# huttered40/capital

Hardware: AMD Instinct MI355X
Metric: TFLOP/s (whole node) Cholesky n=65536, algorithmic n^3/3, recursive cholinv factor(), inputs resident in HBM (higher is better)
Workload: dtype f64

## Files before the change

capital_amd/csrc/equil_f64.hip:

```cpp
#include <float.h>
#include <limits.h>

#include "capi_internal.h"
#include "thin_tile.h"

namespace {

namespace tt = thin_tile;
using tt::d2_t;

__device__ __forceinline__ int scale_exponent(double s) { return (int)((__double_as_longlong(s) >> 52) & 0x7ff) - 1023; }

constexpr int PQ_THREADS = 1024;

__device__ __forceinline__ int frexp_exponent(double a) {
  const unsigned long long b = (unsigned long long)__double_as_longlong(a);
  const int E = (int)((b >> 52) & 0x7ff);
  if (E != 0) return E - 1022;
  return (63 - __clzll((long long)(b & 0xfffffffffffffULL))) - 1073;
}

__global__ __launch_bounds__(PQ_THREADS) void poequ2_kernel(int64_t n, const double* __restrict__ A, int64_t lda, double* __restrict__ dscale,
                                                            double* __restrict__ rec) {
  __shared__ int s_emin[16], s_emax[16];
  __shared__ double s_amin[16], s_amax[16];
  __shared__ long long s_bad[16];
  const int tid = threadIdx.x, lane = tid & 63, w = tid >> 6;
  int emin = INT_MAX, emax = INT_MIN;
  double amin = DBL_MAX, amax = 0.0;
  long long bad = LLONG_MAX;
  for (int64_t j = tid; j < n; j += PQ_THREADS) {
    const double a = A[j + j * lda];
    if (!(a > 0.0) || !(a <= DBL_MAX)) { bad = bad < j ? bad : (long long)j; continue; }
    const int e = frexp_exponent(a) >> 1;
    emin = e < emin ? e : emin; emax = e > emax ? e : emax;
    amin = a < amin ? a : amin; amax = a > amax ? a : amax;
  }
#pragma unroll
  for (int d = 1; d < 64; d <<= 1) {
    const int e0 = __shfl_xor(emin, d), e1 = __shfl_xor(emax, d);
    const double a0 = __shfl_xor(amin, d), a1 = __shfl_xor(amax, d);
    const long long b = __shfl_xor(bad, d);
    emin = e0 < emin ? e0 : emin; emax = e1 > emax ? e1 : emax;
    amin = a0 < amin ? a0 : amin; amax = a1 > amax ? a1 : amax;
    bad = b < bad ? b : bad;
  }
  if (lane == 0) { s_emin[w] = emin; s_emax[w] = emax; s_amin[w] = amin; s_amax[w] = amax; s_bad[w] = bad; }
  __syncthreads();
  for (int k = 0; k < 16; ++k) {
    emin = s_emin[k] < emin ? s_emin[k] : emin; emax = s_emax[k] > emax ? s_emax[k] : emax;
    amin = s_amin[k] < amin ? s_amin[k] : amin; amax = s_amax[k] > amax ? s_amax[k] : amax;
    bad = s_bad[k] < bad ? s_bad[k] : bad;
  }
  const bool ok = bad == LLONG_MAX;
  for (int64_t j = tid; j < n; j += PQ_THREADS) {
    double s = 1.0;
    if (ok) s = __longlong_as_double((long long)((frexp_exponent(A[j + j * lda]) >> 1) + 1023) << 52);
    dscale[j] = s;
  }
  if (tid == 0) {
    rec[0] = ok ? ldexp(1.0, emin - emax) : 1.0;
    rec[1] = ok ? amax : 0.0;
    rec[2] = ok ? amin : 0.0;
    rec[3] = ok ? 0.0 : (double)(bad + 1);
  }
}

constexpr int SC_THREADS = 256;
constexpr int SC_ROWS = 512, SC_COLS = 64, SC_PASS = 8;
constexpr int SC_K = SC_ROWS / SC_COLS;

__host__ __device__ inline int64_t tiles_before(int64_t J) {
  const int64_t q = J / SC_K, s = J % SC_K;
  return SC_K * q * (q + 1) / 2 + s * (q + 1);
}

template <bool VEC>
__global__ __launch_bounds__(SC_THREADS) void sym_scale2_kernel(int64_t n, double* __restrict__ A, int64_t lda, const double* __restrict__ dscale, int sign) {
  const int tid = threadIdx.x;
  const int64_t t = blockIdx.x;
  int64_t q = (int64_t)((sqrt(1.0 + 8.0 * (double)t / SC_K) - 1.0) * 0.5);
  while (q > 0 && SC_K * q * (q + 1) / 2 > t) --q;
  while (SC_K * (q + 1) * (q + 2) / 2 <= t) ++q;
  const int64_t rem = t - SC_K * q * (q + 1) / 2;
  const int64_t J = SC_K * q + rem / (q + 1), I = rem % (q + 1);
  const int64_t i0 = I * SC_ROWS, j0 = J * SC_COLS;
  const bool whole = i0 + SC_ROWS <= j0 + 1 && j0 + SC_COLS <= n;
  if (whole) {
    if (VEC) {
      const int64_t i = i0 + 2 * tid;
      const int ei0 = scale_exponent(dscale[i]), ei1 = scale_exponent(dscale[i + 1]);
      for (int64_t c = j0; c < j0 + SC_COLS; c += SC_PASS) {
        d2_t v[SC_PASS];
#pragma unroll
        for (int p = 0; p < SC_PASS; ++p) v[p] = *(const d2_t*)(A + i + (c + p) * lda);
#pragma unroll
        for (int p = 0; p < SC_PASS; ++p) {
          const int ej = scale_exponent(dscale[c + p]);
          v[p].x = ldexp(v[p].x, -sign * (ei0 + ej));
          v[p].y = ldexp(v[p].y, -sign * (ei1 + ej));
        }
#pragma unroll
        for (int p = 0; p < SC_PASS; ++p) *(d2_t*)(A + i + (c + p) * lda) = v[p];
      }
    } else {
      const int64_t i = i0 + tid;
      const int ei0 = scale_exponent(dscale[i]), ei1 = scale_exponent(dscale[i + SC_THREADS]);
      for (int64_t c = j0; c < j0 + SC_COLS; c += SC_PASS) {
        double x[SC_PASS], y[SC_PASS];
#pragma unroll
        for (int p = 0; p < SC_PASS; ++p) { x[p] = A[i + (c + p) * lda]; y[p] = A[i + SC_THREADS + (c + p) * lda]; }
#pragma unroll
        for (int p = 0; p < SC_PASS; ++p) {
          const int ej = scale_exponent(dscale[c + p]);
          x[p] = ldexp(x[p], -sign * (ei0 + ej));
          y[p] = ldexp(y[p], -sign * (ei1 + ej));
        }
#pragma unroll
        for (int p = 0; p < SC_PASS; ++p) { A[i + (c + p) * lda] = x[p]; A[i + SC_THREADS + (c + p) * lda] = y[p]; }
      }
    }
    return;
  }
  const int64_t ra = i0 + tid, rb = ra + SC_THREADS;
  const int ea = scale_exponent(dscale[ra < n ? ra : 0]), eb = scale_exponent(dscale[rb < n ? rb : 0]);
  for (int64_t c = j0; c < j0 + SC_COLS && c < n; c += SC_PASS) {
    if (i0 + (tid & ~63) > c + SC_PASS - 1) continue;
    double x[SC_PASS], y[SC_PASS];
    bool va[SC_PASS], vb[SC_PASS];
#pragma unroll
    for (int p = 0; p < SC_PASS; ++p) {
      const int64_t col = c + p;
      va[p] = col < n && ra <= col;
      vb[p] = col < n && rb <= col;
      x[p] = *(va[p] ? A + ra + col * lda : A);
      y[p] = *(vb[p] ? A + rb + col * lda : A);
    }
#pragma unroll
    for (int p = 0; p < SC_PASS; ++p) {
      const int ej = scale_exponent(dscale[c + p < n ? c + p : 0]);
      x[p] = ldexp(x[p], -sign * (ea + ej));
      y[p] = ldexp(y[p], -sign * (eb + ej));
    }
#pragma unroll
    for (int p = 0; p < SC_PASS; ++p) {
      if (va[p]) A[ra + (c + p) * lda] = x[p];
      if (vb[p]) A[rb + (c + p) * lda] = y[p];
    }
  }
}

constexpr int RS_THREADS = 256;

__global__ __launch_bounds__(RS_THREADS) void row_scale2_kernel(int64_t m, const double* __restrict__ dscale, int sign, const double* X, int64_t ldx, double* Y,
                                                                int64_t ldy, double* __restrict__ norm2) {
  __shared__ double red[4];
  const double* x = X + (int64_t)blockIdx.x * ldx;
  double* y = Y + (int64_t)blockIdx.x * ldy;
  double s = 0.0;
  for (int64_t i = threadIdx.x; i < m; i += RS_THREADS) {
    const double v = ldexp(x[i], sign * scale_exponent(dscale[i]));
    y[i] = v;
    s += v * v;
  }
  if (!norm2) return;
  s = tt::butterfly_sum<64>(s);
  if ((threadIdx.x & 63) == 0) red[threadIdx.x >> 6] = s;
  __syncthreads();
  if (threadIdx.x == 0) norm2[blockIdx.x] = ((red[0] + red[1]) + red[2]) + red[3];
}

}

extern "C" {

int capi_dpoequ2(capi_handle_t h, int64_t n, const double* A, int64_t lda, double* dscale, double* rec) {
  CAPI_REQUIRE(h, h, "null handle");
  CAPI_REQUIRE(h, n >= 0 && n < (1LL << 31), "n");
  if (n == 0) return CAPI_OK;
  CAPI_REQUIRE(h, A && lda >= n && dscale && rec, "A / lda >= n / dscale / rec");
  hipLaunchKernelGGL(poequ2_kernel, dim3(1), dim3(PQ_THREADS), 0, h->stream, n, A, lda, dscale, rec);
  CAPI_HIP_CHECK(h, hipGetLastError());
  return CAPI_OK;
}

int capi_dsym_scale2(capi_handle_t h, int64_t n, double* A, int64_t lda, const double* dscale, int sign) {
  CAPI_REQUIRE(h, h, "null handle");
  CAPI_REQUIRE(h, n >= 0 && n < (1LL << 31), "n");
  CAPI_REQUIRE(h, sign == 1 || sign == -1, "sign: +1 scales, -1 undoes");
  if (n == 0) return CAPI_OK;
  CAPI_REQUIRE(h, A && lda >= n && dscale, "A / lda >= n / dscale");
  const int64_t tiles = tiles_before(cdiv(n, SC_COLS));
  CAPI_REQUIRE(h, tiles < (1LL << 31), "n too large");
  const bool vec = ((uintptr_t)A & 15) == 0 && (lda & 1) == 0;
  if (vec) hipLaunchKernelGGL(sym_scale2_kernel<true>, dim3((unsigned)tiles), dim3(SC_THREADS), 0, h->stream, n, A, lda, dscale, sign);
  else hipLaunchKernelGGL(sym_scale2_kernel<false>, dim3((unsigned)tiles), dim3(SC_THREADS), 0, h->stream, n, A, lda, dscale, sign);
  CAPI_HIP_CHECK(h, hipGetLastError());
  return CAPI_OK;
}

int capi_drow_scale2(capi_handle_t h, int64_t m, int64_t r, const double* dscale, int sign, const double* X, int64_t ldx, double* Y, int64_t ldy, double* norm2) {
  CAPI_REQUIRE(h, h, "null handle");
  CAPI_REQUIRE(h, m >= 0 && r >= 0 && r < (1LL << 31), "m / r");
  CAPI_REQUIRE(h, sign == 1 || sign == -1, "sign: +1 multiplies by dscale, -1 divides");
  if (r == 0 || m == 0) return CAPI_OK;
  CAPI_REQUIRE(h, dscale && X && Y && ldx >= m && ldy >= m, "dscale / X / Y / ldx >= m / ldy >= m");
  hipLaunchKernelGGL(row_scale2_kernel, dim3((unsigned)r), dim3(RS_THREADS), 0, h->stream, m, dscale, sign, X, ldx, Y, ldy, norm2);
  CAPI_HIP_CHECK(h, hipGetLastError());
  return CAPI_OK;
}

}
```

capital_amd/csrc/movement.hip:

```cpp
#include "capi_internal.h"

namespace {

__device__ __host__ inline int64_t st_offset(int st, int64_t x, int64_t y, int64_t dimY) {
  if (st == CAPI_RECT) return x * dimY + y;
  if (st == CAPI_UPPERTRI) return ((x * (x + 1)) >> 1) + y;
  return x * dimY + y - (x * (x + 1) / 2);
}

__global__ void serialize_kernel(int shape, int ss, int ds, const double* __restrict__ src, int64_t sdimY, double* __restrict__ dst,
                                 int64_t ddimY, int64_t ssx, int64_t ssy, int64_t dsx, int64_t dsy, int64_t rangeX,
                                 int64_t rangeY) {
  const int64_t y = (int64_t)blockIdx.x * 1024 + threadIdx.x;
  const bool lower = shape == CAPI_LOWERTRI, upper = shape == CAPI_UPPERTRI;
  for (int64_t i = blockIdx.y; i < rangeX; i += gridDim.y) {
    int64_t so, d_o, cnt;
    if (lower) {
      so = st_offset(ss, ssx + i, ssy + i, sdimY);
      d_o = st_offset(ds, dsx + i, dsy + i, ddimY);
      cnt = rangeY - i;
    } else {
      so = st_offset(ss, ssx + i, ssy, sdimY);
      d_o = st_offset(ds, dsx + i, dsy, ddimY);
      cnt = upper ? i + 1 : rangeY;
    }
    if (y >= cnt) continue;
    double v[4];
#pragma unroll
    for (int q = 0; q < 4; ++q) v[q] = src[so + (y + 256 * q < cnt ? y + 256 * q : y)];
#pragma unroll
    for (int q = 0; q < 4; ++q)
      if (y + 256 * q < cnt) dst[d_o + y + 256 * q] = v[q];
  }
}

__global__ void lacpy_kernel(int part, int64_t m, int64_t n, const double* __restrict__ A, int64_t lda, double* __restrict__ B,
                             int64_t ldb) {
  const int64_t i = (int64_t)blockIdx.x * blockDim.x + threadIdx.x;
  const int64_t j0 = (int64_t)blockIdx.y * 8;
  if (i >= m) return;
#pragma unroll
  for (int q = 0; q < 8; ++q) {
    const int64_t j = j0 + q;
    if (j >= n) break;
    if (part == 1 && i > j) continue;
    if (part == 2 && i < j) continue;
    B[i + j * ldb] = A[i + j * lda];
  }
}

typedef double d2m_t __attribute__((ext_vector_type(2)));
template <bool VEC>
__global__ __launch_bounds__(256) void copy2d_kernel(int64_t m, int64_t n, const double* __restrict__ A, int64_t lda, double* __restrict__ B, int64_t ldb) {
  const int64_t i = ((int64_t)blockIdx.x * 256 + threadIdx.x) * (VEC ? 2 : 1);
  if (i >= m) return;
  for (int64_t j0 = (int64_t)blockIdx.y * 8; j0 < n; j0 += (int64_t)gridDim.y * 8) {
    if (VEC) {
      d2m_t v[8];
#pragma unroll
      for (int q = 0; q < 8; ++q) v[q] = *(const d2m_t*)(A + i + (j0 + q < n ? j0 + q : j0) * lda);
#pragma unroll
      for (int q = 0; q < 8; ++q)
        if (j0 + q < n) *(d2m_t*)(B + i + (j0 + q) * ldb) = v[q];
    } else {
      double v[8];
#pragma unroll
      for (int q = 0; q < 8; ++q) v[q] = A[i + (j0 + q < n ? j0 + q : j0) * lda];
#pragma unroll
      for (int q = 0; q < 8; ++q)
        if (j0 + q < n) B[i + (j0 + q) * ldb] = v[q];
    }
  }
}

__global__ void geadd_kernel(int part, int64_t m, int64_t n, double alpha, const double* __restrict__ X, int64_t ldx, double beta,
                             double* __restrict__ Y, int64_t ldy) {
  const int64_t i = (int64_t)blockIdx.x * blockDim.x + threadIdx.x;
  if (i >= m) return;
  for (int64_t j = blockIdx.y; j < n; j += gridDim.y) {
    if (part == 1 && i > j) continue;
    if (part == 2 && i < j) continue;
    const double x = alpha == 0.0 ? 0.0 : alpha * X[i + j * ldx];
    Y[i + j * ldy] = beta == 0.0 ? x : x + beta * Y[i + j * ldy];
  }
}

__global__ void trizero_kernel(int keep_uplo, int64_t n, double* __restrict__ A, int64_t lda) {
  const int64_t i = (int64_t)blockIdx.x * blockDim.x + threadIdx.x;
  if (i >= n) return;
  for (int64_t j = blockIdx.y; j < n; j += gridDim.y)
    if (keep_uplo == CAPI_UPPER ? (i > j) : (i < j)) A[i + j * lda] = 0.0;
}

__global__ void axpby_kernel(int64_t count, double beta, const double* __restrict__ x, double* __restrict__ y) {
  int64_t i = (int64_t)blockIdx.x * blockDim.x + threadIdx.x;
  const int64_t stride = (int64_t)gridDim.x * blockDim.x;
  for (; i < count; i += stride) y[i] = beta * y[i] + x[i];
}

__global__ void remove_triangle_kernel(int dirU, double* __restrict__ A, int64_t dimX, int64_t dimY, int64_t px, int64_t py,
                                       int64_t P) {
  const int64_t j = (int64_t)blockIdx.x * blockDim.x + threadIdx.x;
  if (j >= dimY) return;
  for (int64_t i = blockIdx.y; i < dimX; i += gridDim.y) {
    const int64_t gx = px + i * P, gy = py + j * P;
    if (dirU ? (gy > gx) : (gy < gx)) A[i * dimY + j] = 0.0;
  }
}

__global__ void block_cyclic_kernel(int to_cyclic, double* __restrict__ blocked, double* __restrict__ cyclic, int64_t rl,
                                    int64_t cl, int64_t d) {
  const int64_t grow = (int64_t)blockIdx.x * blockDim.x + threadIdx.x;
  const int64_t rg = rl * d, cg = cl * d;
  if (grow >= rg) return;
  for (int64_t gcol = blockIdx.y; gcol < cg; gcol += gridDim.y) {
    const int64_t i = gcol / d, x = gcol % d, k = grow / d, y = grow % d;
    const int64_t b = (y * d + x) * rl * cl + i * rl + k;
    if (to_cyclic == 2) cyclic[gcol * rg + grow] = blocked[b];
    else if (to_cyclic) cyclic[gcol * rg + grow] = (grow > gcol) ? 0.0 : blocked[b];
    else blocked[b] = cyclic[gcol * rg + grow];
  }
}

__global__ void block_cyclic_tri_kernel(int to_cyclic, double* __restrict__ blocked, double* __restrict__ cyclic, int64_t rl, int64_t d) {
  const int64_t grow = (int64_t)blockIdx.x * blockDim.x + threadIdx.x;
  const int64_t rg = rl * d, psz = rl * (rl + 1) / 2;
  if (grow >= rg) return;
  for (int64_t gcol = blockIdx.y; gcol < rg; gcol += gridDim.y) {
    const int64_t i = gcol / d, x = gcol % d, k = grow / d, y = grow % d;
    if (k > i) { if (to_cyclic) cyclic[gcol * rg + grow] = 0.0; continue; }
    const int64_t b = (y * d + x) * psz + i * (i + 1) / 2 + k;
    const bool below = grow > gcol;
    if (to_cyclic) cyclic[gcol * rg + grow] = below ? 0.0 : blocked[b];
    else blocked[b] = below ? 0.0 : cyclic[gcol * rg + grow];
  }
}

__global__ void cyclic_to_local_kernel(int pass, double* __restrict__ T, double* __restrict__ TI, double* __restrict__ tmp, int64_t L, int64_t bc,
                                       int64_t d, int64_t ro, int64_t co) {
  const int64_t j = (int64_t)blockIdx.x * blockDim.x + threadIdx.x;
  if (j >= L) return;
  for (int64_t i = blockIdx.y; i < L; i += gridDim.y) {
    const int64_t rc = i * d + co, rr = j * d + ro;
    if (pass == 0) {
      tmp[i * L + j] = rc >= rr ? T[rc * bc + rr] : 0.0;
      tmp[L * L + i * L + j] = rc >= rr ? TI[rc * bc + rr] : 0.0;
    } else {
      T[i * bc + j] = tmp[i * L + j];
      TI[i * bc + j] = tmp[L * L + i * L + j];
    }
  }
}

constexpr uint64_t LCG_A = 0x5DEECE66DULL, LCG_C = 0xBULL, LCG_MASK = (1ULL << 48) - 1;

__device__ __forceinline__ uint64_t seed48(int64_t seed) { return ((((uint64_t)seed) & 0xffffffffULL) << 16) | 0x330EULL; }
__device__ __forceinline__ double to_unit(uint64_t x) { return (double)x * 0x1p-48; }

__global__ void gen_symmetric_kernel(double* __restrict__ data, int64_t dimX, int64_t dimY, int64_t gdimX, int64_t gdimY,
                                     int64_t px, int64_t py, int64_t PX, int64_t PY, int64_t padX, int64_t padY, int dd) {
  const int64_t j = (int64_t)blockIdx.x * blockDim.x + threadIdx.x;
  if (j >= dimY) return;
  for (int64_t i = blockIdx.y; i < dimX; i += gridDim.y) {
    double v = 0.0;
    if (i < padX && j < padY) {
      const int64_t gx = px + i * PX, gy = py + j * PY;
      const int64_t seed = gx > gy ? gx + gdimY * gy : gy + gdimY * gx;
      const uint64_t x1 = (LCG_A * seed48(seed) + LCG_C) & LCG_MASK;
      v = to_unit(x1);
      if (dd && gx == gy && i == j) v += (double)gdimX;
    }
    data[i * dimY + j] = v;
  }
}

constexpr int GEN_CHUNK = 32;
__global__ void gen_random_kernel(double* __restrict__ data, int64_t dimX, int64_t dimY, int64_t padX, int64_t padY, int64_t key) {
  const int64_t chunk = (int64_t)blockIdx.x * blockDim.x + threadIdx.x;
  const int64_t total = padX * padY;
  int64_t t0 = chunk * GEN_CHUNK;
  if (t0 >= total) return;
  uint64_t An = 1, Cn = 0, Ab = LCG_A, Cb = LCG_C;
  for (uint64_t n = (uint64_t)t0; n; n >>= 1) {
    if (n & 1) { An = (Ab * An) & LCG_MASK; Cn = (Ab * Cn + Cb) & LCG_MASK; }
    Cb = (Ab * Cb + Cb) & LCG_MASK;
    Ab = (Ab * Ab) & LCG_MASK;
  }
  uint64_t x = (An * seed48(key) + Cn) & LCG_MASK;
  const int64_t t1 = (t0 + GEN_CHUNK < total) ? t0 + GEN_CHUNK : total;
  for (int64_t t = t0; t < t1; ++t) {
    x = (LCG_A * x + LCG_C) & LCG_MASK;
    const int64_t i = t / padY, j = t - i * padY;
    data[i * dimY + j] = to_unit(x);
  }
}

__global__ void gen_pad_zero_kernel(double* __restrict__ data, int64_t dimX, int64_t dimY, int64_t padX, int64_t padY) {
  const int64_t j = (int64_t)blockIdx.x * blockDim.x + threadIdx.x;
  if (j >= dimY) return;
  for (int64_t i = blockIdx.y; i < dimX; i += gridDim.y)
    if (i >= padX || j >= padY) data[i * dimY + j] = 0.0;
}

__global__ void gen_identity_kernel(double* __restrict__ data, int64_t dimX, int64_t dimY, int64_t px, int64_t py, int64_t PX,
                                    int64_t PY, int64_t padX, int64_t padY, double val) {
  const int64_t j = (int64_t)blockIdx.x * blockDim.x + threadIdx.x;
  if (j >= dimY) return;
  for (int64_t i = blockIdx.y; i < dimX; i += gridDim.y) {
    double v = 0.0;
    if (i < padX && j < padY && (px + i * PX == py + j * PY) && i == j) v = val;
    data[i * dimY + j] = v;
  }
}

__global__ void diff_norms_kernel(int part, int64_t m, int64_t n, const double* __restrict__ X, int64_t ldx,
                                  const double* __restrict__ Y, int64_t ldy, double* __restrict__ partial) {
  __shared__ double se[256], sc[256];
  const int64_t j = blockIdx.x;
  double e = 0.0, c = 0.0;
  for (int64_t i = threadIdx.x; i < m; i += 256) {
    if (part == 1 && i > j) break;
    if (part == 2 && i < j) continue;
    const double y = Y[i + j * ldy], dlt = X[i + j * ldx] - y;
    e += dlt * dlt;
    c += y * y;
  }
  se[threadIdx.x] = e;
  sc[threadIdx.x] = c;
  __syncthreads();
  for (int s = 128; s > 0; s >>= 1) {
    if (threadIdx.x < s) { se[threadIdx.x] += se[threadIdx.x + s]; sc[threadIdx.x] += sc[threadIdx.x + s]; }
    __syncthreads();
  }
  if (threadIdx.x == 0) { partial[2 * j] = se[0]; partial[2 * j + 1] = sc[0]; }
}

void pad_lens(int64_t dimX, int64_t dimY, int64_t gdimX, int64_t gdimY, int64_t px, int64_t py, int64_t PX, int64_t PY,
              int64_t* padX, int64_t* padY) {
  *padX = (((gdimX % PX != 0) && ((dimX - 1) * PX + px >= gdimX)) ? dimX - 1 : dimX);
  *padY = (((gdimY % PY != 0) && ((dimY - 1) * PY + py >= gdimY)) ? dimY - 1 : dimY);
}

inline dim3 grid2(int64_t rows, int64_t cols) { return dim3((unsigned)cdiv(rows, 256), (unsigned)(cols < 65535 ? cols : 65535)); }

}

extern "C" {

int capi_serialize_shape(capi_handle_t h, int shape, int ss, int ds, const double* src, int64_t sdimX, int64_t sdimY, double* dst,
                         int64_t ddimX, int64_t ddimY, int64_t ssx, int64_t sex, int64_t ssy, int64_t sey, int64_t dsx, int64_t dex,
                         int64_t dsy, int64_t dey) {
  CAPI_REQUIRE(h, h, "null handle");
  CAPI_REQUIRE(h, ss >= 0 && ss <= 2 && ds >= 0 && ds <= 2 && shape >= 0 && shape <= 2, "structure code");
  CAPI_REQUIRE(h, (sex - ssx) == (dex - dsx) && (sey - ssy) == (dey - dsy), "source and destination ranges differ");
  (void)sdimX; (void)ddimX;
  const int64_t rangeX = sex - ssx, rangeY = sey - ssy;
  if (rangeX <= 0 || rangeY <= 0) return CAPI_OK;
  CAPI_REQUIRE(h, src && dst, "null matrix");
  hipLaunchKernelGGL(serialize_kernel, dim3((unsigned)cdiv(rangeY, 1024), (unsigned)(rangeX < 65535 ? rangeX : 65535)), dim3(256), 0, h->stream, shape, ss, ds, src, sdimY, dst, ddimY, ssx, ssy,
                     dsx, dsy, rangeX, rangeY);
  CAPI_HIP_CHECK(h, hipGetLastError());
  return CAPI_OK;
}

int capi_serialize(capi_handle_t h, int ss, int ds, const double* src, int64_t sdimX, int64_t sdimY, double* dst, int64_t ddimX,
                   int64_t ddimY, int64_t ssx, int64_t sex, int64_t ssy, int64_t sey, int64_t dsx, int64_t dex, int64_t dsy,
                   int64_t dey) {
  const int shape = (ss == CAPI_LOWERTRI || ds == CAPI_LOWERTRI) ? CAPI_LOWERTRI : ((ss == CAPI_UPPERTRI || ds == CAPI_UPPERTRI) ? CAPI_UPPERTRI : CAPI_RECT);
  return capi_serialize_shape(h, shape, ss, ds, src, sdimX, sdimY, dst, ddimX, ddimY, ssx, sex, ssy, sey, dsx, dex, dsy, dey);
}

__attribute__((visibility("hidden"))) int capi_internal_copy2d(capi_handle_t h, int64_t m, int64_t n, const double* A, int64_t lda, double* B, int64_t ldb) {
  if (m <= 0 || n <= 0 || (A == B && lda == ldb)) return CAPI_OK;
  if (lda == m && ldb == m && m * n >= (1 << 16) && (m > 8192 || n == 1)) {
    const int64_t total = m * n, cols = total / 8192, rest = total - cols * 8192;
    int rc = capi_internal_copy2d(h, 8192, cols, A, 8192, B, 8192);
    if (rc != CAPI_OK || rest == 0) return rc;
    return capi_internal_copy2d(h, rest, 1, A + cols * 8192, rest, B + cols * 8192, rest);
  }
  const bool vec = (((uintptr_t)A | (uintptr_t)B) & 15) == 0 && ((lda | ldb | m) & 1) == 0;
  const int64_t gx = cdiv(vec ? m / 2 : m, 256), gy = cdiv(n, 8);
  CAPI_REQUIRE(h, gx < (1LL << 31), "copy too tall");
  const dim3 grid((unsigned)gx, (unsigned)(gy < 65535 ? gy : 65535));
  if (vec) hipLaunchKernelGGL(copy2d_kernel<true>, grid, dim3(256), 0, h->stream, m, n, A, lda, B, ldb);
  else hipLaunchKernelGGL(copy2d_kernel<false>, grid, dim3(256), 0, h->stream, m, n, A, lda, B, ldb);
  CAPI_HIP_CHECK(h, hipGetLastError());
  return CAPI_OK;
}

int capi_dlacpy(capi_handle_t h, int part, int64_t m, int64_t n, const double* A, int64_t lda, double* B, int64_t ldb) {
  CAPI_REQUIRE(h, h, "null handle");
  CAPI_REQUIRE(h, part >= 0 && part <= 2 && m >= 0 && n >= 0, "args");
  if (m == 0 || n == 0) return CAPI_OK;
  CAPI_REQUIRE(h, A && B && lda >= m && ldb >= m, "operands");
  if (part == 0) return capi_internal_copy2d(h, m, n, A, lda, B, ldb);
  const int64_t gy = cdiv(n, 8);
  CAPI_REQUIRE(h, gy <= 65535, "n too large");
  hipLaunchKernelGGL(lacpy_kernel, dim3((unsigned)cdiv(m, 256), (unsigned)gy), dim3(256), 0, h->stream, part, m, n, A, lda, B, ldb);
  CAPI_HIP_CHECK(h, hipGetLastError());
  return CAPI_OK;
}

int capi_dgeadd(capi_handle_t h, int part, int64_t m, int64_t n, double alpha, const double* X, int64_t ldx, double beta, double* Y,
                int64_t ldy) {
  CAPI_REQUIRE(h, h, "null handle");
  CAPI_REQUIRE(h, part >= 0 && part <= 2 && m >= 0 && n >= 0, "args");
  if (m == 0 || n == 0) return CAPI_OK;
  CAPI_REQUIRE(h, X && Y && ldx >= m && ldy >= m, "operands");
  hipLaunchKernelGGL(geadd_kernel, grid2(m, n), dim3(256), 0, h->stream, part, m, n, alpha, X, ldx, beta, Y, ldy);
  CAPI_HIP_CHECK(h, hipGetLastError());
  return CAPI_OK;
}

int capi_dtrizero(capi_handle_t h, int keep_uplo, int64_t n, double* A, int64_t lda) {
  CAPI_REQUIRE(h, h, "null handle");
  CAPI_REQUIRE(h, (keep_uplo == 0 || keep_uplo == 1) && n >= 0, "args");
  if (n == 0) return CAPI_OK;
  CAPI_REQUIRE(h, A && lda >= n, "A/lda");
  hipLaunchKernelGGL(trizero_kernel, grid2(n, n), dim3(256), 0, h->stream, keep_uplo, n, A, lda);
  CAPI_HIP_CHECK(h, hipGetLastError());
  return CAPI_OK;
}

int capi_daxpby(capi_handle_t h, int64_t count, double beta, const double* x, double* y) {
  CAPI_REQUIRE(h, h, "null handle");
  if (count <= 0) return count < 0 ? CAPI_EINVAL : CAPI_OK;
  CAPI_REQUIRE(h, x && y, "null vector");
  int64_t blocks = cdiv(count, 256);
  if (blocks > h->num_cu * 16) blocks = h->num_cu * 16;
  hipLaunchKernelGGL(axpby_kernel, dim3((unsigned)blocks), dim3(256), 0, h->stream, count, beta, x, y);
  CAPI_HIP_CHECK(h, hipGetLastError());
  return CAPI_OK;
}

int capi_remove_triangle(capi_handle_t h, char dir, double* A, int64_t dimX, int64_t dimY, int64_t px, int64_t py, int64_t P) {
  CAPI_REQUIRE(h, h, "null handle");
  CAPI_REQUIRE(h, (dir == 'U' || dir == 'L') && dimX >= 0 && dimY >= 0 && P > 0, "args");
  if (dimX == 0 || dimY == 0) return CAPI_OK;
  hipLaunchKernelGGL(remove_triangle_kernel, grid2(dimY, dimX), dim3(256), 0, h->stream, dir == 'U', A, dimX, dimY, px, py, P);
  CAPI_HIP_CHECK(h, hipGetLastError());
  return CAPI_OK;
}

int capi_block_to_cyclic(capi_handle_t h, const double* blocked, double* cyclic, int64_t rl, int64_t cl, int64_t d) {
  CAPI_REQUIRE(h, h && blocked && cyclic && rl > 0 && cl > 0 && d > 0, "args");
  hipLaunchKernelGGL(block_cyclic_kernel, grid2(rl * d, cl * d), dim3(256), 0, h->stream, 1, (double*)blocked, cyclic, rl, cl, d);
  CAPI_HIP_CHECK(h, hipGetLastError());
  return CAPI_OK;
}
int capi_block_to_cyclic_full(capi_handle_t h, const double* blocked, double* cyclic, int64_t rl, int64_t cl, int64_t d) {
  CAPI_REQUIRE(h, h && blocked && cyclic && rl > 0 && cl > 0 && d > 0, "args");
  hipLaunchKernelGGL(block_cyclic_kernel, grid2(rl * d, cl * d), dim3(256), 0, h->stream, 2, (double*)blocked, cyclic, rl, cl, d);
  CAPI_HIP_CHECK(h, hipGetLastError());
  return CAPI_OK;
}

int capi_cyclic_to_block(capi_handle_t h, double* blocked, const double* cyclic, int64_t rl, int64_t cl, int64_t d) {
  CAPI_REQUIRE(h, h && blocked && cyclic && rl > 0 && cl > 0 && d > 0, "args");
  hipLaunchKernelGGL(block_cyclic_kernel, grid2(rl * d, cl * d), dim3(256), 0, h->stream, 0, blocked, (double*)cyclic, rl, cl, d);
  CAPI_HIP_CHECK(h, hipGetLastError());
  return CAPI_OK;
}

int capi_block_to_cyclic_tri(capi_handle_t h, const double* blocked, double* cyclic, int64_t rl, int64_t d) {
  CAPI_REQUIRE(h, h && blocked && cyclic && rl > 0 && d > 0, "args");
  hipLaunchKernelGGL(block_cyclic_tri_kernel, grid2(rl * d, rl * d), dim3(256), 0, h->stream, 1, (double*)blocked, cyclic, rl, d);
  CAPI_HIP_CHECK(h, hipGetLastError());
  return CAPI_OK;
}
int capi_cyclic_to_block_tri(capi_handle_t h, double* blocked, const double* cyclic, int64_t rl, int64_t d) {
  CAPI_REQUIRE(h, h && blocked && cyclic && rl > 0 && d > 0, "args");
  hipLaunchKernelGGL(block_cyclic_tri_kernel, grid2(rl * d, rl * d), dim3(256), 0, h->stream, 0, blocked, (double*)cyclic, rl, d);
  CAPI_HIP_CHECK(h, hipGetLastError());
  return CAPI_OK;
}

int capi_cyclic_to_local(capi_handle_t h, double* T, double* TI, int64_t local_dim, int64_t bc_dim, int64_t d, int64_t slice_rank) {
  CAPI_REQUIRE(h, h && T && TI && local_dim > 0 && d > 0 && bc_dim >= local_dim * d && slice_rank >= 0 && slice_rank < d * d, "args");
  void* w;
  int rc = capi_ws2_get(h, sizeof(double) * 2 * (size_t)local_dim * (size_t)local_dim, &w);
  if (rc != CAPI_OK) return rc;
  for (int pass = 0; pass < 2; ++pass)
    hipLaunchKernelGGL(cyclic_to_local_kernel, grid2(local_dim, local_dim), dim3(256), 0, h->stream, pass, T, TI, (double*)w, local_dim, bc_dim, d,
                       slice_rank / d, slice_rank % d);
  CAPI_HIP_CHECK(h, hipGetLastError());
  return CAPI_OK;
}

int capi_distribute_symmetric(capi_handle_t h, double* data, int64_t dimX, int64_t dimY, int64_t gdimX, int64_t gdimY, int64_t px,
                              int64_t py, int64_t PX, int64_t PY, int64_t key, int dd) {
  (void)key;
  CAPI_REQUIRE(h, h && data && dimX > 0 && dimY > 0 && PX > 0 && PY > 0, "args");
  int64_t padX, padY;
  pad_lens(dimX, dimY, gdimX, gdimY, px, py, PX, PY, &padX, &padY);
  hipLaunchKernelGGL(gen_symmetric_kernel, grid2(dimY, dimX), dim3(256), 0, h->stream, data, dimX, dimY, gdimX, gdimY, px, py, PX, PY,
                     padX, padY, dd);
  CAPI_HIP_CHECK(h, hipGetLastError());
  return CAPI_OK;
}

int capi_distribute_random(capi_handle_t h, double* data, int64_t dimX, int64_t dimY, int64_t gdimX, int64_t gdimY, int64_t px,
                           int64_t py, int64_t PX, int64_t PY, int64_t key) {
  CAPI_REQUIRE(h, h && data && dimX > 0 && dimY > 0 && PX > 0 && PY > 0, "args");
  int64_t padX, padY;
  pad_lens(dimX, dimY, gdimX, gdimY, px, py, PX, PY, &padX, &padY);
  if (padX != dimX || padY != dimY) {
    hipLaunchKernelGGL(gen_pad_zero_kernel, grid2(dimY, dimX), dim3(256), 0, h->stream, data, dimX, dimY, padX, padY);
    CAPI_HIP_CHECK(h, hipGetLastError());
  }
  const int64_t chunks = cdiv(padX * padY, GEN_CHUNK);
  if (chunks > 0) {
    hipLaunchKernelGGL(gen_random_kernel, dim3((unsigned)cdiv(chunks, 256)), dim3(256), 0, h->stream, data, dimX, dimY, padX, padY, key);
    CAPI_HIP_CHECK(h, hipGetLastError());
  }
  return CAPI_OK;
}

int capi_distribute_identity(capi_handle_t h, double* data, int64_t dimX, int64_t dimY, int64_t gdimX, int64_t gdimY, int64_t px,
                             int64_t py, int64_t PX, int64_t PY, double val) {
  CAPI_REQUIRE(h, h && data && dimX > 0 && dimY > 0 && PX > 0 && PY > 0, "args");
  int64_t padX, padY;
  pad_lens(dimX, dimY, gdimX, gdimY, px, py, PX, PY, &padX, &padY);
  hipLaunchKernelGGL(gen_identity_kernel, grid2(dimY, dimX), dim3(256), 0, h->stream, data, dimX, dimY, px, py, PX, PY, padX, padY, val);
  CAPI_HIP_CHECK(h, hipGetLastError());
  return CAPI_OK;
}

int capi_diff_norms(capi_handle_t h, int part, int64_t m, int64_t n, const double* X, int64_t ldx, const double* Y, int64_t ldy,
                    double* out2) {
  CAPI_REQUIRE(h, h && out2 && part >= 0 && part <= 2 && m >= 0 && n >= 0, "args");
  out2[0] = out2[1] = 0.0;
  if (m == 0 || n == 0) return CAPI_OK;
  CAPI_REQUIRE(h, X && Y && ldx >= m && ldy >= m, "operands");
  void* w;
  int rc = capi_ws_get(h, sizeof(double) * 2 * (size_t)n, &w);
  if (rc != CAPI_OK) return rc;
  hipLaunchKernelGGL(diff_norms_kernel, dim3((unsigned)n), dim3(256), 0, h->stream, part, m, n, X, ldx, Y, ldy, (double*)w);
  CAPI_HIP_CHECK(h, hipGetLastError());
  double* host = (double*)malloc(sizeof(double) * 2 * (size_t)n);
  if (!host) return CAPI_ENOMEM;
  rc = capi_memcpy_d2h(h, host, w, sizeof(double) * 2 * (size_t)n);
  if (rc == CAPI_OK)
    for (int64_t j = 0; j < n; ++j) { out2[0] += host[2 * j]; out2[1] += host[2 * j + 1]; }
  free(host);
  return rc;
}

}
```

Before: 55.49.

## Add tiled triangular copy kernel for serialize and dlacpy

Factors the triangular tile-index mapping into a shared header and adds a tiled copy kernel. Each 256-thread block moves a 512x64 tile using paired 16-byte loads and stores, with a lane-shuffle fallback when the destination is only 8-byte aligned. Large serialize (rect/upper) and triangular dlacpy calls now use it instead of the older per-element kernels. For upper shapes, tiles are enumerated only over the triangle, so no blocks are launched for the empty half. Small copies keep the old path, and the edge-tile handling adds complexity and correctness risk.

```diff
diff --git a/capital_amd/csrc/equil_f64.hip b/capital_amd/csrc/equil_f64.hip
--- a/capital_amd/csrc/equil_f64.hip
+++ b/capital_amd/csrc/equil_f64.hip
@@ -3,6 +3,7 @@
 
 #include "capi_internal.h"
 #include "thin_tile.h"
+#include "tri_tiles.h"
 
 namespace {
 
@@ -66,24 +67,15 @@
   }
 }
 
-constexpr int SC_THREADS = 256;
-constexpr int SC_ROWS = 512, SC_COLS = 64, SC_PASS = 8;
-constexpr int SC_K = SC_ROWS / SC_COLS;
-
-__host__ __device__ inline int64_t tiles_before(int64_t J) {
-  const int64_t q = J / SC_K, s = J % SC_K;
-  return SC_K * q * (q + 1) / 2 + s * (q + 1);
-}
+constexpr int SC_THREADS = tri_tiles::TRI_THREADS;
+constexpr int SC_ROWS = tri_tiles::TRI_ROWS, SC_COLS = tri_tiles::TRI_COLS, SC_PASS = tri_tiles::TRI_PASS;
+using tri_tiles::tiles_before;
 
 template <bool VEC>
 __global__ __launch_bounds__(SC_THREADS) void sym_scale2_kernel(int64_t n, double* __restrict__ A, int64_t lda, const double* __restrict__ dscale, int sign) {
   const int tid = threadIdx.x;
-  const int64_t t = blockIdx.x;
-  int64_t q = (int64_t)((sqrt(1.0 + 8.0 * (double)t / SC_K) - 1.0) * 0.5);
-  while (q > 0 && SC_K * q * (q + 1) / 2 > t) --q;
-  while (SC_K * (q + 1) * (q + 2) / 2 <= t) ++q;
-  const int64_t rem = t - SC_K * q * (q + 1) / 2;
-  const int64_t J = SC_K * q + rem / (q + 1), I = rem % (q + 1);
+  int64_t I, J;
+  tri_tiles::tile_of(blockIdx.x, &I, &J);
   const int64_t i0 = I * SC_ROWS, j0 = J * SC_COLS;
   const bool whole = i0 + SC_ROWS <= j0 + 1 && j0 + SC_COLS <= n;
   if (whole) {
diff --git a/capital_amd/csrc/movement.hip b/capital_amd/csrc/movement.hip
--- a/capital_amd/csrc/movement.hip
+++ b/capital_amd/csrc/movement.hip
@@ -1,4 +1,5 @@
 #include "capi_internal.h"
+#include "tri_tiles.h"
 
 namespace {
 
@@ -73,6 +74,78 @@
   }
 }
 
+enum { TC_RECT = 0, TC_UPPER = 1, TC_LOWER = 2 };
+constexpr int64_t TRI_COPY_MIN = 256;
+struct tri_copy_args {
+  const double* src;
+  double* dst;
+  int64_t sdimY, ddimY, sx0, sy0, dx0, dy0, nx, ny, row_tiles;
+  int shape, ss, ds;
+};
+__device__ __forceinline__ int64_t tc_col(int st, int64_t x, int64_t dimY) { return st == CAPI_RECT ? x * dimY : (x * (x + 1)) >> 1; }
+
+template <bool LD16>
+__global__ __launch_bounds__(tri_tiles::TRI_THREADS) void tri_copy_kernel(const tri_copy_args a) {
+  using namespace tri_tiles;
+  const int tid = threadIdx.x;
+  int64_t I, J;
+  if (a.shape == TC_UPPER) tile_of(blockIdx.x, &I, &J);
+  else { I = (int64_t)blockIdx.x % a.row_tiles; J = (int64_t)blockIdx.x / a.row_tiles; }
+  const int64_t i0 = I * TRI_ROWS, j0 = J * TRI_COLS;
+  if (i0 >= a.ny) return;
+  if (a.shape == TC_LOWER && i0 + TRI_ROWS <= j0) return;
+  const double* __restrict__ const S = a.src + a.sy0;
+  double* __restrict__ const D = a.dst + a.dy0;
+  bool whole = j0 + TRI_COLS <= a.nx && i0 + TRI_ROWS <= a.ny;
+  if (a.shape == TC_UPPER) whole = whole && i0 + TRI_ROWS <= j0 + 1;
+  if (a.shape == TC_LOWER) whole = whole && i0 >= j0 + TRI_COLS - 1;
+  if (whole) {
+    const int64_t i = i0 + 2 * tid;
+    for (int64_t c = j0 + (int64_t)blockIdx.y * TRI_PASS; c < j0 + TRI_COLS; c += (int64_t)gridDim.y * TRI_PASS) {
+      d2m_t v[TRI_PASS];
+#pragma unroll
+      for (int p = 0; p < TRI_PASS; ++p) {
+        const double* s = S + tc_col(a.ss, a.sx0 + c + p, a.sdimY) + i;
+        if (LD16) v[p] = *(const d2m_t*)s;
+        else { v[p].x = s[0]; v[p].y = s[1]; }
+      }
+#pragma unroll
+      for (int p = 0; p < TRI_PASS; ++p) {
+        double* d = D + tc_col(a.ds, a.dx0 + c + p, a.ddimY) + i;
+        if (((uintptr_t)d & 15) == 0) { *(d2m_t*)d = v[p]; continue; }
+        const double below = __shfl_down(v[p].x, 1);
+        const int lane = tid & 63;
+        if (lane < 63) { d2m_t w; w.x = v[p].y; w.y = below; *(d2m_t*)(d + 1) = w; }
+        if (lane == 0 || lane == 63) d[lane == 0 ? 0 : 1] = lane == 0 ? v[p].x : v[p].y;
+      }
+    }
+    return;
+  }
+  const int64_t ra = i0 + tid, rb = ra + TRI_THREADS;
+  const double* const first = S + tc_col(a.ss, a.sx0, a.sdimY);
+  for (int64_t c = j0 + (int64_t)blockIdx.y * TRI_PASS; c < j0 + TRI_COLS && c < a.nx; c += (int64_t)gridDim.y * TRI_PASS) {
+    if (a.shape == TC_UPPER && i0 + (tid & ~63) > c + TRI_PASS - 1) continue;
+    double x[TRI_PASS], y[TRI_PASS];
+    bool va[TRI_PASS], vb[TRI_PASS];
+#pragma unroll
+    for (int p = 0; p < TRI_PASS; ++p) {
+      const int64_t col = c + p;
+      const int64_t lo = a.shape == TC_LOWER ? col : 0, hi = a.shape == TC_UPPER && col + 1 < a.ny ? col + 1 : a.ny;
+      va[p] = col < a.nx && ra >= lo && ra < hi;
+      vb[p] = col < a.nx && rb >= lo && rb < hi;
+      const double* s = S + tc_col(a.ss, a.sx0 + (col < a.nx ? col : 0), a.sdimY);
+      x[p] = *(va[p] ? s + ra : first);
+      y[p] = *(vb[p] ? s + rb : first);
+    }
+#pragma unroll
+    for (int p = 0; p < TRI_PASS; ++p) {
+      double* d = D + tc_col(a.ds, a.dx0 + c + p, a.ddimY);
+      if (va[p]) d[ra] = x[p];
+      if (vb[p]) d[rb] = y[p];
+    }
+  }
+}
+
 __global__ void geadd_kernel(int part, int64_t m, int64_t n, double alpha, const double* __restrict__ X, int64_t ldx, double beta,
                              double* __restrict__ Y, int64_t ldy) {
   const int64_t i = (int64_t)blockIdx.x * blockDim.x + threadIdx.x;
@@ -243,6 +316,20 @@
 
 inline dim3 grid2(int64_t rows, int64_t cols) { return dim3((unsigned)cdiv(rows, 256), (unsigned)(cols < 65535 ? cols : 65535)); }
 
+int tri_copy(capi_handle_t h, tri_copy_args a) {
+  if (a.nx <= 0 || a.ny <= 0) return CAPI_OK;
+  a.row_tiles = cdiv(a.ny, tri_tiles::TRI_ROWS);
+  const int64_t col_tiles = cdiv(a.nx, tri_tiles::TRI_COLS);
+  const int64_t tiles = a.shape == TC_UPPER ? tri_tiles::tiles_before(col_tiles) : a.row_tiles * col_tiles;
+  CAPI_REQUIRE(h, tiles < (1LL << 31), "copy too large");
+  const bool ld16 = a.ss == CAPI_RECT && (a.sdimY & 1) == 0 && ((uintptr_t)(a.src + a.sx0 * a.sdimY + a.sy0) & 15) == 0;
+  const dim3 grid((unsigned)tiles, tiles <= 16 ? tri_tiles::TRI_COLS / tri_tiles::TRI_PASS : 1);
+  if (ld16) hipLaunchKernelGGL(tri_copy_kernel<true>, grid, dim3(tri_tiles::TRI_THREADS), 0, h->stream, a);
+  else hipLaunchKernelGGL(tri_copy_kernel<false>, grid, dim3(tri_tiles::TRI_THREADS), 0, h->stream, a);
+  CAPI_HIP_CHECK(h, hipGetLastError());
+  return CAPI_OK;
+}
+
 }
 
 extern "C" {
@@ -257,6 +344,11 @@
   const int64_t rangeX = sex - ssx, rangeY = sey - ssy;
   if (rangeX <= 0 || rangeY <= 0) return CAPI_OK;
   CAPI_REQUIRE(h, src && dst, "null matrix");
+  if (shape != CAPI_LOWERTRI && ss != CAPI_LOWERTRI && ds != CAPI_LOWERTRI && (rangeX > TRI_COPY_MIN || rangeY > TRI_COPY_MIN)) {
+    tri_copy_args a{src, dst, sdimY, ddimY, ssx, ssy, dsx, dsy, rangeX, shape == CAPI_UPPERTRI ? rangeX : rangeY, 0,
+                    shape == CAPI_UPPERTRI ? TC_UPPER : TC_RECT, ss, ds};
+    return tri_copy(h, a);
+  }
   hipLaunchKernelGGL(serialize_kernel, dim3((unsigned)cdiv(rangeY, 1024), (unsigned)(rangeX < 65535 ? rangeX : 65535)), dim3(256), 0, h->stream, shape, ss, ds, src, sdimY, dst, ddimY, ssx, ssy,
                      dsx, dsy, rangeX, rangeY);
   CAPI_HIP_CHECK(h, hipGetLastError());
@@ -294,11 +386,13 @@
   if (m == 0 || n == 0) return CAPI_OK;
   CAPI_REQUIRE(h, A && B && lda >= m && ldb >= m, "operands");
   if (part == 0) return capi_internal_copy2d(h, m, n, A, lda, B, ldb);
-  const int64_t gy = cdiv(n, 8);
-  CAPI_REQUIRE(h, gy <= 65535, "n too large");
-  hipLaunchKernelGGL(lacpy_kernel, dim3((unsigned)cdiv(m, 256), (unsigned)gy), dim3(256), 0, h->stream, part, m, n, A, lda, B, ldb);
-  CAPI_HIP_CHECK(h, hipGetLastError());
-  return CAPI_OK;
+  if (m <= TRI_COPY_MIN && n <= TRI_COPY_MIN) {
+    hipLaunchKernelGGL(lacpy_kernel, dim3((unsigned)cdiv(m, 256), (unsigned)cdiv(n, 8)), dim3(256), 0, h->stream, part, m, n, A, lda, B, ldb);
+    CAPI_HIP_CHECK(h, hipGetLastError());
+    return CAPI_OK;
+  }
+  tri_copy_args a{A, B, lda, ldb, 0, 0, 0, 0, n, m, 0, part == 1 ? TC_UPPER : TC_LOWER, CAPI_RECT, CAPI_RECT};
+  return tri_copy(h, a);
 }
 
 int capi_dgeadd(capi_handle_t h, int part, int64_t m, int64_t n, double alpha, const double* X, int64_t ldx, double beta, double* Y,
diff --git a/capital_amd/csrc/tri_tiles.h b/capital_amd/csrc/tri_tiles.h
--- /dev/null
+++ b/capital_amd/csrc/tri_tiles.h
@@ -0,0 +1,29 @@
+#ifndef CAPITAL_TRI_TILES_H_
+#define CAPITAL_TRI_TILES_H_
+
+#include <stdint.h>
+#include <math.h>
+
+namespace tri_tiles {
+
+constexpr int TRI_THREADS = 256;
+constexpr int TRI_ROWS = 512, TRI_COLS = 64, TRI_PASS = 8;
+constexpr int TRI_K = TRI_ROWS / TRI_COLS;
+
+__host__ __device__ inline int64_t tiles_before(int64_t J) {
+  const int64_t q = J / TRI_K, s = J % TRI_K;
+  return TRI_K * q * (q + 1) / 2 + s * (q + 1);
+}
+
+__device__ inline void tile_of(int64_t t, int64_t* I, int64_t* J) {
+  int64_t q = (int64_t)((sqrt(1.0 + 8.0 * (double)t / TRI_K) - 1.0) * 0.5);
+  while (q > 0 && TRI_K * q * (q + 1) / 2 > t) --q;
+  while (TRI_K * (q + 1) * (q + 2) / 2 <= t) ++q;
+  const int64_t rem = t - TRI_K * q * (q + 1) / 2;
+  *J = TRI_K * q + rem / (q + 1);
+  *I = rem % (q + 1);
+}
+
+}
+
+#endif
```

Result: no change. 55.52 (median of 2 runs) (+0.1%).
